# owensgroup/sparsify.me

Measured on AMD Instinct MI355X. Metric: effective GF/s (2:4 spmma vs dense gemm) on ResNet-50 layer shapes, higher is better.
Workload: dtype f16

## Files before the change

sparsify.me_amd/csrc/spmma_f16_fused.hip:

```cpp
#include "select24.h"
#include "spmma_args.h"

namespace sm {

constexpr int MAXG = 8;
struct FusedArgs {
  const half_t* A[MAXG];
  const half_t* B[MAXG];
  half_t* C[MAXG];
  size_t sA, sB, sC;
  int Mrows, N, K, lda;
  int batch, tiles_m, tiles_n;
  int ngroup;
  float alpha, beta;
  const half_t* const* dAp;
  const half_t* const* dBp;
  half_t* const* dCp;
};

template <int BN, int NS, bool BF = false, int BM = 128, int NWV = 4, bool ANT = true, bool DENSE = false>
__global__ __launch_bounds__(64 * NWV, (BN == 128 && NWV == 4 && BM == 128) ? 4 : 1) void spmma_f16_fused_direct_kernel(const FusedArgs p) {
  static_assert(BM == 128 || BM == 64, "row tile");
  static_assert(NWV == 4 || (NWV == 8 && BM == 128), "waves per workgroup");
  constexpr int NW = NWV, TM = BM / NW, FM = TM / 16, FN = BN / 16;
// ... 979 lines not shown
        strip_select_f16(src[i][0], src[i][1], k0, n0);
        strip_select_f16(src[i][2], src[i][3], k1, n1);
        *reinterpret_cast<u2*>(sb + a_val_off[i]) = u2{k0, k1};
        *reinterpret_cast<unsigned char*>(sb + a_meta_off[i]) = (unsigned char)(n0 | (n1 << 4));
      }
    };
    auto step = [&](int g, u4 (&rr)[4], bool write, bool load) {
      asm volatile("s_waitcnt lgkmcnt(0)\n\ts_barrier" ::: "memory");
      __builtin_amdgcn_sched_barrier(0);
      if (write) write_stage(g + 1, rr);
      if (load) load_a(rr);
      __builtin_amdgcn_sched_barrier(0);
    };
    int g0 = 0;
    if (S > 2 * PF) {
#pragma unroll
      for (int s = 0; s < PF; ++s) load_a(ra[s]);
      write_stage(0, ra[0]);
      load_a(ra[0]);
      for (; g0 + 2 * PF < S; g0 += PF) {
#pragma unroll
        for (int u = 0; u < PF; ++u) step(g0 + u, ra[(u + 1) % PF], true, true);
      }
    } else {
#pragma unroll
      for (int s = 0; s < PF; ++s)
        if (s < S) load_a(ra[s]);
      write_stage(0, ra[0]);
      if (PF < S) load_a(ra[0]);
    }
    for (; g0 < S; g0 += PF) {
#pragma unroll
      for (int u = 0; u < PF; ++u) {
        const int g = g0 + u;
        if (g < S) step(g, ra[(u + 1) % PF], g + 1 < S, g + 1 + PF < S);
      }
    }
  } else {
    const unsigned g4 = lane >> 4, r = lane & 15u;
    const unsigned wm = wave / WN, wn = wave % WN;
    char* const patch = smem + CPATCH + wave * WPATCH;
    f4 acc[FM][FN];
#pragma unroll
    for (int i = 0; i < FM; ++i)
#pragma unroll
      for (int j = 0; j < FN; ++j) acc[i][j] = f4{0.f, 0.f, 0.f, 0.f};
    int cb = 0, kt = 0;
    unsigned cj = 0;
    Tile t = tile_of(0);
    for (int g = 0; g < S; ++g) {
      asm volatile("s_barrier" ::: "memory");
      const char* As = smem + (g & 1) * ASTG;
      smfmac_stage<FM, FN, BF>(As, As + SA, smem + BRING + cb * SB, wm * TM, wn * TN, lane, acc);
      cb = cb + 1 == NSB ? 0 : cb + 1;
      if (++kt == nkt) {
        half_t* C = p.C[t.grp] + (size_t)t.b * p.sC;
        const bool c_vec = (reinterpret_cast<uintptr_t>(C) & 15u) == 0 && (p.N % 8 == 0);
        if (p.beta == 0.0f && c_vec) {
#pragma unroll
          for (int h = 0; h < 2; ++h) {
#pragma unroll
            for (int i = 0; i < FM; ++i)
#pragma unroll
              for (int j = 0; j < FN / 2; ++j) {
                const unsigned lr = i * 16 + 4u * g4, lc = j * 16 + r;
#pragma unroll
                for (int q = 0; q < 4; ++q)
                  *reinterpret_cast<half_t*>(patch + (lr + q) * WPITCH + lc * 2) = to_elt<BF>(p.alpha * acc[i][h * (FN / 2) + j][q]);
              }
            asm volatile("s_waitcnt lgkmcnt(0)" ::: "memory");
            const int gc = t.n0 + (int)(wn * TN) + 64 * h + 8 * (int)(lane & 7u);
#pragma unroll
            for (int s8 = 0; s8 < TM / 8; ++s8) {
              const unsigned lr = 8u * s8 + (lane >> 3);
              const int gr = t.m0 + (int)(wm * TM + lr);
              if (gr < p.Mrows && gc < p.N) {
                const u2 lo = *reinterpret_cast<const u2*>(patch + lr * WPITCH + 16u * (lane & 7u));
                const u2 hi = *reinterpret_cast<const u2*>(patch + lr * WPITCH + 16u * (lane & 7u) + 8u);
                __builtin_nontemporal_store(u4{lo[0], lo[1], hi[0], hi[1]}, reinterpret_cast<u4*>(C + (size_t)gr * p.N + gc));
              }
            }
            asm volatile("s_waitcnt lgkmcnt(0)" ::: "memory");
          }
        } else {
#pragma unroll
          for (int i = 0; i < FM; ++i)
#pragma unroll
            for (int j = 0; j < FN; ++j) {
              const int gc = t.n0 + (int)(wn * TN + j * 16 + r);
              if (gc >= p.N) continue;
#pragma unroll
              for (int q = 0; q < 4; ++q) {
                const int gr = t.m0 + (int)(wm * TM + i * 16 + 4u * g4) + q;
                if (gr >= p.Mrows) continue;
                half_t* dst = C + (size_t)gr * p.N + gc;
                float v = p.alpha * acc[i][j][q];
                if (p.beta != 0.0f) v += p.beta * to_f32<BF>(*dst);
                *dst = to_elt<BF>(v);
              }
            }
        }
#pragma unroll
        for (int i = 0; i < FM; ++i)
#pragma unroll
          for (int j = 0; j < FN; ++j) acc[i][j] = f4{0.f, 0.f, 0.f, 0.f};
        kt = 0;
        if (++cj < my_tiles) t = tile_of(cj);
      }
    }
  }
}

template <int BN, int WM, int WN, int NLB, int PF, int NSB, bool BF = false>
static int launch_fused_widep(const FusedArgs& a0, hipStream_t st) {
  FusedArgs a = a0;
  a.tiles_m = (a.Mrows + 127) / 128;
  a.tiles_n = (a.N + BN - 1) / BN;
  const size_t nt = (size_t)a.tiles_m * a.tiles_n * a.batch * a.ngroup;
  if (nt == 0) return SM_STATUS_SUCCESS;
  if (nt > 0x7fffffffu) {
    set_error("sm_spmma_fused_f16: grid too large");
    return SM_STATUS_NOT_SUPPORTED;
  }
  constexpr size_t lds = 2 * (size_t)128 * 72 + (size_t)NSB * 64 * BN * 2 + (size_t)(WM * WN) * 32 * (64 * 2 + 8);
  static_assert(lds <= 160 * 1024, "LDS budget of the persistent wide kernel");
  static LdsOptIn lds_optin;
  if (const int rc = ensure_dyn_lds(lds_optin, reinterpret_cast<const void*>(&spmma_f16_fused_widep_kernel<BN, WM, WN, NLB, PF, NSB, BF>), lds, "spmma_f16_fused_widep_kernel")) return rc;
  size_t cus = (size_t)device_cu_count();
  cus -= cus % 8;
  if (cus == 0) cus = 8;
  const unsigned grid = (unsigned)(nt <= cus ? nt : cus);
  spmma_f16_fused_widep_kernel<BN, WM, WN, NLB, PF, NSB, BF><<<dim3(grid), dim3(64 * (WM * WN + 4 + NLB)), lds, st>>>(a, (unsigned)nt);
  return check_launch("spmma_f16_fused_widep_kernel");
}

template <int NSB, bool BF = false>
__global__ __launch_bounds__(64 * 16) void spmma_f16_fused_astat_kernel(const FusedArgs p, int nsplit, int tiles_per_split) {
  constexpr int BM = 128, BN = 128, WM = 4, WN = 2, NC = 8, NLA = 4, NLB = 4;
  static_assert(NC + NLA + NLB == 16, "launch bounds");
  constexpr int TM = BM / WM, TN = BN / WN, FM = TM / 16, FN = TN / 16;
  constexpr int SA = BM * 64, SM_ = BM * 8, ASTG = SA + SM_, SB = 64 * BN * 2;
  constexpr int B_N = BN / 8, B_WI = B_N / NLB;
  static_assert((NSB - 2) * B_WI <= 63, "vmcnt range");
  constexpr int WPITCH = TN * 2 + 8, WPATCH = TM * WPITCH;
  extern __shared__ __attribute__((aligned(16))) char smem[];

  const unsigned tid = threadIdx.x, lane = tid & 63u;
  const unsigned wave = __builtin_amdgcn_readfirstlane(tid >> 6);
  const int nkt = p.K / 64;
  const unsigned per_batch = (unsigned)p.tiles_m * (unsigned)nsplit;
  const unsigned lid = xcd_remap(blockIdx.x, gridDim.x);
  const unsigned gb = lid / per_batch, trem = lid - gb * per_batch;
  const unsigned grp = gb / (unsigned)p.batch, b = gb - grp * (unsigned)p.batch;
  const unsigned tile_m = trem / (unsigned)nsplit, split = trem - tile_m * (unsigned)nsplit;
  const int m0 = (int)tile_m * BM;
  const int nt0 = (int)split * tiles_per_split;
  const int nt1 = nt0 + tiles_per_split < p.tiles_n ? nt0 + tiles_per_split : p.tiles_n;
  const int T = (nt1 - nt0) * nkt;
  char* const Bring = smem + nkt * ASTG;
  char* const Cpatch = Bring + NSB * SB;
  half_t* C = p.C[grp] + (size_t)b * p.sC;

  const bool is_b = wave >= (unsigned)(NC + NLA);
  const unsigned lwb = is_b ? wave - (NC + NLA) : 0u;
  const char* Bb = reinterpret_cast<const char*>(p.B[grp] + (size_t)b * p.sB);
  unsigned b_kr[B_WI], b_col[B_WI], b_dst[B_WI];
#pragma unroll
  for (int i = 0; i < B_WI; ++i) {
    const unsigned j = lwb + (unsigned)NLB * i, panel = j >> 3, grp = j & 7u, kr = 8u * grp + (lane >> 3);
    b_kr[i] = kr;
    b_col[i] = 64u * panel + 8u * ((lane & 7u) ^ b_swz(kr));
    b_dst[i] = panel * 8192u + grp * 1024u;
  }
  const size_t row_bytes = (size_t)p.N * 2;
  int i_nt = nt0, i_kt = 0, i_buf = 0;
  auto issue_b = [&]() {
#pragma unroll
    for (int i = 0; i < B_WI; ++i) {
      int gc = i_nt * BN + (int)b_col[i];
      gc = gc <= p.N - 8 ? gc : p.N - 8;
      const char* src = Bb + (size_t)(i_kt * 64 + (int)b_kr[i]) * row_bytes + (size_t)gc * 2;
      __builtin_amdgcn_global_load_lds((gptr_t*)src, (lptr_t*)(Bring + i_buf * SB + b_dst[i]), 16, 0, 0);
    }
    i_buf = i_buf + 1 == NSB ? 0 : i_buf + 1;
    if (++i_kt == nkt) { i_kt = 0; ++i_nt; }
  };
  if (is_b) {
#pragma unroll
    for (int s = 0; s < NSB - 1; ++s)
      if (s < T) issue_b();
  }

  {
    const half_t* A = p.A[grp] + (size_t)b * p.sA;
    const unsigned row = 8u * wave + (lane >> 3), c8 = lane & 7u;
    int gr = m0 + (int)row;
    gr = gr < p.Mrows - 1 ? gr : p.Mrows - 1;
    const half_t* a_src = A + (size_t)gr * p.lda + 8u * c8;
    const unsigned a_val_off = row * 64u + 16u * ((c8 >> 1) ^ a64_swz(row)) + 8u * (c8 & 1u);
    const unsigned a_meta_off = SA + row * 8u + c8;
    u4 ra[8];
#pragma unroll
    for (int s = 0; s < 8; ++s)
      if (s < nkt) ra[s] = __builtin_nontemporal_load(reinterpret_cast<const u4*>(a_src + (size_t)s * 64));
#pragma unroll
    for (int s = 0; s < 8; ++s)
      if (s < nkt) {
        uint32_t k0, k1, n0, n1;
        strip_select_f16(ra[s][0], ra[s][1], k0, n0);
        strip_select_f16(ra[s][2], ra[s][3], k1, n1);
        char* sb = smem + s * ASTG;
        *reinterpret_cast<u2*>(sb + a_val_off) = u2{k0, k1};
        *reinterpret_cast<unsigned char*>(sb + a_meta_off) = (unsigned char)(n0 | (n1 << 4));
      }
  }
  __syncthreads();
  if (wave >= (unsigned)NC && !is_b) {
    for (int it = 0; it < T; ++it) asm volatile("s_barrier" ::: "memory");
    return;
  }

  if (is_b) {
    for (int it = 0; it < T; ++it) {
      if (it + NSB - 2 < T) wait_dma_and_barrier<(NSB - 2) * B_WI>();
      else wait_dma_and_barrier<0>();
      if (it + NSB - 1 < T) issue_b();
    }
  } else {
    const unsigned g = lane >> 4, r = lane & 15u;
    const unsigned wm = wave / WN, wn = wave % WN;
    char* const patch = Cpatch + wave * WPATCH;
    f4 acc[FM][FN];
#pragma unroll
    for (int i = 0; i < FM; ++i)
#pragma unroll
      for (int j = 0; j < FN; ++j) acc[i][j] = f4{0.f, 0.f, 0.f, 0.f};
    int cb = 0, kt = 0, nt = nt0;
    for (int it = 0; it < T; ++it) {
      asm volatile("s_barrier" ::: "memory");
      const char* As = smem + kt * ASTG;
      const char* Ms = As + SA;
      const char* Bs = Bring + cb * SB;
      smfmac_stage<FM, FN, BF>(As, Ms, Bs, wm * TM, wn * TN, lane, acc);
      cb = cb + 1 == NSB ? 0 : cb + 1;
      if (++kt == nkt) {
#pragma unroll
        for (int i = 0; i < FM; ++i)
#pragma unroll
          for (int j = 0; j < FN; ++j) {
            const unsigned lr = i * 16 + 4u * g, lc = j * 16 + r;
#pragma unroll
            for (int q = 0; q < 4; ++q) {
              *reinterpret_cast<half_t*>(patch + (lr + q) * WPITCH + lc * 2) = to_elt<BF>(p.alpha * acc[i][j][q]);
              acc[i][j][q] = 0.f;
            }
          }
        asm volatile("s_waitcnt lgkmcnt(0)" ::: "memory");
        const int gc = nt * BN + (int)(wn * TN) + 8 * (int)(lane & 7u);
#pragma unroll
        for (int s = 0; s < TM / 8; ++s) {
          const unsigned lr = 8u * s + (lane >> 3);
          const int gr = m0 + (int)(wm * TM + lr);
          if (gr < p.Mrows && gc < p.N) {
            const u2 lo = *reinterpret_cast<const u2*>(patch + lr * WPITCH + 16u * (lane & 7u));
            const u2 hi = *reinterpret_cast<const u2*>(patch + lr * WPITCH + 16u * (lane & 7u) + 8u);
            __builtin_nontemporal_store(u4{lo[0], lo[1], hi[0], hi[1]}, reinterpret_cast<u4*>(C + (size_t)gr * p.N + gc));
          }
        }
        kt = 0;
        ++nt;
      }
    }
  }
}


static size_t astat_lds_bytes(int nkt, int nsb) { return (size_t)nkt * (128 * 72) + (size_t)nsb * 64 * 128 * 2 + 8 * 32 * (64 * 2 + 8); }

template <bool BF = false>
static int launch_fused_astat(const FusedArgs& a0, hipStream_t st) {
  FusedArgs a = a0;
  a.tiles_m = (a.Mrows + 127) / 128;
  a.tiles_n = (a.N + 127) / 128;
  const int cus = device_cu_count();
  const size_t panels = (size_t)a.tiles_m * a.batch * a.ngroup;
  int nsplit = 1;
  while (panels * nsplit * 4 < (size_t)3 * cus && (a.tiles_n + 2 * nsplit - 1) / (2 * nsplit) >= 2) nsplit *= 2;
  int tps = (a.tiles_n + nsplit - 1) / nsplit;
  nsplit = (a.tiles_n + tps - 1) / tps;
  const size_t nwg = panels * nsplit;
  if (nwg == 0) return SM_STATUS_SUCCESS;
  if (nwg > 0x7fffffffu) {
    set_error("sm_spmma_fused_f16: grid too large");
    return SM_STATUS_NOT_SUPPORTED;
  }
  constexpr int NSB = 3;
  const size_t lds = astat_lds_bytes(a.K / 64, NSB);
  static LdsOptIn lds_optin;
  if (const int rc = ensure_dyn_lds(lds_optin, reinterpret_cast<const void*>(&spmma_f16_fused_astat_kernel<NSB, BF>), (160 * 1024), "spmma_f16_fused_astat_kernel")) return rc;
  spmma_f16_fused_astat_kernel<NSB, BF><<<dim3((unsigned)nwg), dim3(64 * 16), lds, st>>>(a, nsplit, tps);
  return check_launch("spmma_f16_fused_astat_kernel");
}

}

using namespace sm;

static bool span_form_takes(size_t m, size_t n, size_t k, size_t lda, size_t batch, size_t strideA, size_t strideB, size_t strideC, bool all_aligned, bool c_aligned) {
  return (k % 64 != 0 || lda % 8 != 0) && lda == k && n % 8 == 0 && n <= 128 && all_aligned && c_aligned && (batch == 1 || (strideB == 0 && strideA == m * lda && strideC == m * n)) &&
         (m * batch * k * 2) % 16 == 0 && m * batch <= 0x7fffffffull && k <= 0x7fffffffull &&
         ((size_t)128 * k * 2 + 1152) + ((k + 63) / 64 * 64) * (n <= 64 ? 64 : 128) * 2 <= 160 * 1024;
}
static bool stage_forms_take(size_t n, size_t k, size_t lda, size_t strideA, size_t strideB, bool all_aligned) {
  return !(k % 64 != 0 || lda % 8 != 0 || strideA % 8 != 0 || n % 8 != 0 || strideB % 8 != 0 || !all_aligned);
}
static bool dims_fit_int(size_t m, size_t n, size_t k, size_t lda, size_t batch) {
  return !(m * batch > 0x7fffffffull || n > 0x7fffffffull || k > 0x7fffffffull || lda > 0x7fffffffull);
}
bool sm::spmma_fused16_takes_exact(const void* A, const void* B, const void* C, size_t m, size_t n, size_t k, size_t lda, size_t batch, size_t strideA, size_t strideB,
                                   size_t strideC) {
  if (!A || !B || !C || lda < k || m == 0 || n == 0 || batch == 0) return false;
  if (n < 8 && k <= 64) return false;
  const bool all_aligned = aligned16(A) && aligned16(B), c_aligned = aligned16(C);
  if (span_form_takes(m, n, k, lda, batch, strideA, strideB, strideC, all_aligned, c_aligned)) return true;
  return stage_forms_take(n, k, lda, strideA, strideB, all_aligned) && dims_fit_int(m, n, k, lda, batch);
}

template <bool BF>
static int spmma_fused16(size_t ngroup, const void* const* Ag, const void* const* Bg, void* const* Cg, size_t m, size_t n, size_t k, size_t lda,
                         size_t batch, size_t strideA, size_t strideB, size_t strideC, float alpha, float beta,
                         sm_stream_t stream, void* workspace = nullptr, size_t workspace_bytes = 0) {
  if (ngroup == 0) return SM_STATUS_SUCCESS;
  if (!Ag || !Bg || !Cg || lda < k || ngroup > (size_t)MAXG) {
    set_error("sm_spmma_fused_{f16,bf16}: invalid argument");
    return SM_STATUS_INVALID_VALUE;
  }
  bool all_aligned = true, c_aligned = true;
  for (size_t g = 0; g < ngroup; ++g) {
    if (!Ag[g] || !Bg[g] || !Cg[g]) {
      set_error("sm_spmma_fused_{f16,bf16}: invalid argument (null operand)");
      return SM_STATUS_INVALID_VALUE;
    }
    all_aligned = all_aligned && aligned16(Ag[g]) && aligned16(Bg[g]);
    c_aligned = c_aligned && aligned16(Cg[g]);
  }
  if (m == 0 || n == 0 || batch == 0) return SM_STATUS_SUCCESS;
  if (n < 8 && k <= 64 && lda == k && (batch == 1 || (strideB == 0 && strideA == m * lda && strideC == m * n))) {
    const int rc = spmma_fused_thin(BF, (int)ngroup, Ag, Bg, Cg, m * batch, n, k, alpha, beta, (hipStream_t)stream);
    if (rc != SM_STATUS_NOT_SUPPORTED) return rc;
  }
  if (span_form_takes(m, n, k, lda, batch, strideA, strideB, strideC, all_aligned, c_aligned)) {
    FusedArgs a = {};
    for (size_t g = 0; g < (size_t)MAXG; ++g) {
      const size_t s_ = g < ngroup ? g : 0;
      a.A[g] = (const half_t*)Ag[s_]; a.B[g] = (const half_t*)Bg[s_]; a.C[g] = (half_t*)Cg[s_];
    }
    a.ngroup = (int)ngroup;
    a.Mrows = (int)(m * batch); a.N = (int)n; a.K = (int)k; a.lda = (int)lda;
    a.batch = 1; a.alpha = alpha; a.beta = beta;
    hipStream_t st = (hipStream_t)stream;
    return n <= 64 ? launch_fused_span<64, BF>(a, st) : launch_fused_span<128, BF>(a, st);
  }
  if (!stage_forms_take(n, k, lda, strideA, strideB, all_aligned)) {
    set_error("sm_spmma_fused_{f16,bf16}: needs k %% 64 == 0, n %% 8 == 0 and 16-byte aligned rows (use the staged path)");
    return SM_STATUS_NOT_SUPPORTED;
  }
  if (ngroup > 1 && !c_aligned) {
    set_error("sm_spmma_fused_{f16,bf16}_grouped: needs 16-byte aligned C operands");
    return SM_STATUS_NOT_SUPPORTED;
  }
  if (!dims_fit_int(m, n, k, lda, batch)) {
    set_error("sm_spmma_fused_{f16,bf16}: dimension exceeds 2^31-1");
    return SM_STATUS_NOT_SUPPORTED;
  }
  FusedArgs a = {};
  for (size_t g = 0; g < (size_t)MAXG; ++g) {
    const size_t s_ = g < ngroup ? g : 0;
    a.A[g] = (const half_t*)Ag[s_]; a.B[g] = (const half_t*)Bg[s_]; a.C[g] = (half_t*)Cg[s_];
  }
  a.ngroup = (int)ngroup;
  void* const C = Cg[0];
  a.sA = strideA; a.sB = strideB; a.sC = strideC;
  a.Mrows = (int)m; a.N = (int)n; a.K = (int)k; a.lda = (int)lda;
  a.batch = (int)batch; a.alpha = alpha; a.beta = beta;
  if (batch > 1 && strideB == 0 && strideA == m * lda && strideC == m * n) {
    a.Mrows = (int)(m * batch);
    a.batch = 1;
  }
  hipStream_t st = (hipStream_t)stream;
  auto round_eff = [](size_t tiles, size_t cus) { const size_t r = (tiles + cus - 1) / cus; return r ? (double)tiles / (double)(r * cus) : 1.0; };
  if (workspace) {
    const bool astat_shape = n > 256 && k <= 512 && beta == 0.0f && aligned16(C) && (strideC % 8 == 0);
    SkPlan pl;
    if (sk_takes((size_t)a.Mrows, (size_t)a.batch * a.ngroup, n, k, astat_shape, pl) &&
        workspace_bytes >= sk_workspace_bytes((size_t)pl.slots * ((n + 255) / 256), 256) && aligned16(workspace)) {
      const int rc = n <= 256 ? launch_fused_sk<256, BF, true>(a, workspace, workspace_bytes, st) : launch_fused_sk<256, BF, false>(a, workspace, workspace_bytes, st);
      if (rc != SM_STATUS_NOT_SUPPORTED) return rc;
    }
  }
  if (n > 128 && k > 64) {
    const size_t cus = (size_t)device_cu_count(), nb = (size_t)a.batch * a.ngroup;
    const size_t t_big = ((size_t)a.Mrows + 255) / 256 * ((n + 255) / 256) * nb, t_wide = ((size_t)a.Mrows + 127) / 128 * ((n + 255) / 256) * nb;
    const bool astat_shape = n > 256 && k <= 512 && beta == 0.0f && aligned16(C) && (strideC % 8 == 0);
    bool big = round_eff(t_big, cus) >= round_eff(t_wide, cus);
    if (astat_shape) {
      const size_t panels = ((size_t)a.Mrows + 127) / 128 * nb;
      size_t ns = 1, tn = (n + 127) / 128;
      while (panels * ns * 4 < 3 * cus && (tn + 2 * ns - 1) / (2 * ns) >= 2) ns *= 2;
      big = round_eff(t_big, cus) > round_eff(panels * ns, cus) + 0.1;
    }
    if (big) return n <= 256 ? launch_fused_big<256, BF, 3, 2, true>(a, st) : launch_fused_big<256, BF, 3, 2, false>(a, st);
  }
  if (n <= 128 || (n <= 256 && k <= 64)) {
    if (n <= 64) return launch_fused_direct<64, 2, BF>(a, st);
    if (n > 128 || k < 512) return launch_fused_direct<128, 2, BF, 128, 4, false>(a, st);
    return launch_fused_direct<128, 2, BF>(a, st);
  }
  if (n > 256 && k <= 512 && beta == 0.0f && aligned16(C) && (strideC % 8 == 0) &&
      astat_lds_bytes((int)(k / 64), 3) <= 160 * 1024) {
    return launch_fused_astat<BF>(a, st);
  }
  if (k <= 1024) return launch_fused_widep<256, 4, 2, 4, 2, 3, BF>(a, st);
  if (n > 256) return launch_fused_wide<256, 4, 2, 4, 2, 3, BF, false>(a, st);
  return launch_fused_wide<256, 4, 2, 4, 2, 3, BF>(a, st);
}

extern "C" int sm_spmma_fused_f16(const void* A, const void* B, void* C, size_t m, size_t n, size_t k, size_t lda,
                                  size_t batch, size_t strideA, size_t strideB, size_t strideC, float alpha, float beta,
                                  sm_stream_t stream) {
  return spmma_fused16<false>(1, &A, &B, &C, m, n, k, lda, batch, strideA, strideB, strideC, alpha, beta, stream);
}
extern "C" int sm_spmma_fused_bf16(const void* A, const void* B, void* C, size_t m, size_t n, size_t k, size_t lda,
                                   size_t batch, size_t strideA, size_t strideB, size_t strideC, float alpha, float beta,
                                   sm_stream_t stream) {
  return spmma_fused16<true>(1, &A, &B, &C, m, n, k, lda, batch, strideA, strideB, strideC, alpha, beta, stream);
}

extern "C" int sm_spmma_fused_workspace_size(size_t* bytes) {
  if (!bytes) {
    set_error("sm_spmma_fused_workspace_size: invalid argument");
    return SM_STATUS_INVALID_VALUE;
  }
  *bytes = sk_workspace_bytes((size_t)device_cu_count(), 256);
  return SM_STATUS_SUCCESS;
}
extern "C" int sm_spmma_fused_workspace_state(const void* workspace, int* state, sm_stream_t stream) {
  if (!workspace || !state) {
    set_error("sm_spmma_fused_workspace_state: invalid argument");
    return SM_STATUS_INVALID_VALUE;
  }
  unsigned h[1024];
  hipStream_t st = (hipStream_t)stream;
  if (hipMemcpyAsync(h, workspace, sizeof(h), hipMemcpyDeviceToHost, st) != hipSuccess || hipStreamSynchronize(st) != hipSuccess)
    return check_launch("sm_spmma_fused_workspace_state");
  bool dirty = false;
  for (int i = 0; i < 1023; ++i) dirty = dirty || h[i] != 0u;
  *state = h[1023] != 0u ? 1 : (dirty ? 2 : 0);
  return SM_STATUS_SUCCESS;
}
extern "C" int sm_spmma_fused_streamk_plan(size_t rows, size_t n, size_t k, size_t problems, int* takes, unsigned* plan) {
  if (!takes || !plan) {
    set_error("sm_spmma_fused_streamk_plan: invalid argument");
    return SM_STATUS_INVALID_VALUE;
  }
  SkPlan pl = {};
  *takes = sk_takes(rows, problems, n, k, n > 256 && k <= 512, pl) ? 1 : 0;
  unsigned* o = plan;
  *o++ = pl.tg; *o++ = pl.wg; *o++ = pl.groups_full; *o++ = pl.tgl; *o++ = pl.wgl; *o++ = pl.slots; *o++ = pl.units;
  for (int i = 0; i < 9; ++i) *o++ = pl.cut[i];
  for (int i = 0; i < 9; ++i) *o++ = pl.cutl[i];
  return SM_STATUS_SUCCESS;
}
extern "C" int sm_spmma_fused_f16_ws(const void* A, const void* B, void* C, size_t m, size_t n, size_t k, size_t lda, size_t batch, size_t strideA,
                                     size_t strideB, size_t strideC, float alpha, float beta, void* workspace, size_t workspace_bytes, sm_stream_t stream) {
  return spmma_fused16<false>(1, &A, &B, &C, m, n, k, lda, batch, strideA, strideB, strideC, alpha, beta, stream, workspace, workspace_bytes);
}
extern "C" int sm_spmma_fused_bf16_ws(const void* A, const void* B, void* C, size_t m, size_t n, size_t k, size_t lda, size_t batch, size_t strideA,
                                      size_t strideB, size_t strideC, float alpha, float beta, void* workspace, size_t workspace_bytes, sm_stream_t stream) {
  return spmma_fused16<true>(1, &A, &B, &C, m, n, k, lda, batch, strideA, strideB, strideC, alpha, beta, stream, workspace, workspace_bytes);
}

template <bool BF>
static int dense_twin16(const DenseTwinCall& c, hipStream_t st) {
  const size_t n = (size_t)c.N, k = (size_t)c.K;
  const bool tables = c.Ap != nullptr;
  if (tables != (c.Bp != nullptr) || tables != (c.Cp != nullptr)) return SM_STATUS_NOT_SUPPORTED;
  if (c.N % 8 != 0 || c.N < 8 || (!tables && (!aligned16(c.A) || !aligned16(c.B) || !aligned16(c.C)))) return SM_STATUS_NOT_SUPPORTED;
  FusedArgs a = {};
  for (int g = 0; g < MAXG; ++g) { a.A[g] = c.A; a.B[g] = c.B; a.C[g] = c.C; }
  a.dAp = c.Ap; a.dBp = c.Bp; a.dCp = c.Cp;
  a.ngroup = 1;
  a.sA = c.sA; a.sB = c.sB; a.sC = c.sC;
  a.Mrows = c.M; a.N = c.N; a.K = c.K; a.lda = c.lda;
  a.batch = c.batch; a.alpha = c.alpha; a.beta = c.beta;
  if (k % 64 != 0 || c.lda % 8 != 0) {
    if (c.lda != c.K || n > 128 || ((size_t)c.M * k * 2) % 16 != 0 || (c.batch > 1 && !tables)) return SM_STATUS_NOT_SUPPORTED;
    if (((size_t)128 * k * 2 + 1152) + ((k + 63) / 64 * 64) * (n <= 64 ? 64 : 128) * 2 > 160 * 1024) return SM_STATUS_NOT_SUPPORTED;
    a.ngroup = c.batch;
    a.batch = 1;
    if (!tables) a.ngroup = 1;
    return n <= 64 ? launch_fused_span<64, BF, true>(a, st) : launch_fused_span<128, BF, true>(a, st);
  }
  if (c.sA % 8 != 0 || c.sB % 8 != 0) return SM_STATUS_NOT_SUPPORTED;
  if (c.workspace && n > 128 && n <= 256 && k >= 2048) {
    SkPlan pl;
    if (sk_takes((size_t)c.M, (size_t)c.batch, n, k, false, pl) && c.workspace_bytes >= sk_workspace_bytes((size_t)pl.slots * ((n + 255) / 256), 256) &&
        aligned16(c.workspace))
      return launch_fused_sk<256, BF, true, true>(a, c.workspace, c.workspace_bytes, st);
  }
  if (n <= 128) return SM_STATUS_NOT_SUPPORTED;
  if (k <= 64) return SM_STATUS_NOT_SUPPORTED;
  if (((size_t)c.M + 255) / 256 * 256 * 100 > (size_t)c.M * 115) return SM_STATUS_NOT_SUPPORTED;
  if (!(n <= 256 && k >= 2048)) return SM_STATUS_NOT_SUPPORTED;
  return launch_fused_big<256, BF, 3, 2, true, true>(a, st);
}

int sm::gemm_dense_twin(const DenseTwinCall& c, hipStream_t st) { return c.bf ? dense_twin16<true>(c, st) : dense_twin16<false>(c, st); }

template <bool BF>
static int spmma_fused16_grouped(size_t count, const void* const* A, const void* const* B, void* const* C, size_t m, size_t n, size_t k,
                                 size_t lda, size_t batch, size_t strideA, size_t strideB, size_t strideC, float alpha, float beta,
                                 sm_stream_t stream, void* workspace = nullptr, size_t workspace_bytes = 0) {
  if (count && (!A || !B || !C)) {
    set_error("sm_spmma_fused_{f16,bf16}_grouped: invalid argument");
    return SM_STATUS_INVALID_VALUE;
  }
  for (size_t i = 0; i < count; i += (size_t)MAXG) {
    const size_t ng = count - i < (size_t)MAXG ? count - i : (size_t)MAXG;
    if (const int rc = spmma_fused16<BF>(ng, A + i, B + i, C + i, m, n, k, lda, batch, strideA, strideB, strideC, alpha, beta, stream, workspace, workspace_bytes)) return rc;
  }
  return SM_STATUS_SUCCESS;
}
extern "C" int sm_spmma_fused_f16_grouped(size_t count, const void* const* A, const void* const* B, void* const* C, size_t m, size_t n,
                                          size_t k, size_t lda, size_t batch, size_t strideA, size_t strideB, size_t strideC,
                                          float alpha, float beta, sm_stream_t stream) {
  return spmma_fused16_grouped<false>(count, A, B, C, m, n, k, lda, batch, strideA, strideB, strideC, alpha, beta, stream);
}
extern "C" int sm_spmma_fused_bf16_grouped(size_t count, const void* const* A, const void* const* B, void* const* C, size_t m, size_t n,
                                           size_t k, size_t lda, size_t batch, size_t strideA, size_t strideB, size_t strideC,
                                           float alpha, float beta, sm_stream_t stream) {
  return spmma_fused16_grouped<true>(count, A, B, C, m, n, k, lda, batch, strideA, strideB, strideC, alpha, beta, stream);
}
extern "C" int sm_spmma_fused_f16_grouped_ws(size_t count, const void* const* A, const void* const* B, void* const* C, size_t m, size_t n,
                                             size_t k, size_t lda, size_t batch, size_t strideA, size_t strideB, size_t strideC,
                                             float alpha, float beta, void* workspace, size_t workspace_bytes, sm_stream_t stream) {
  return spmma_fused16_grouped<false>(count, A, B, C, m, n, k, lda, batch, strideA, strideB, strideC, alpha, beta, stream, workspace, workspace_bytes);
}
extern "C" int sm_spmma_fused_bf16_grouped_ws(size_t count, const void* const* A, const void* const* B, void* const* C, size_t m, size_t n,
                                              size_t k, size_t lda, size_t batch, size_t strideA, size_t strideB, size_t strideC,
                                              float alpha, float beta, void* workspace, size_t workspace_bytes, sm_stream_t stream) {
  return spmma_fused16_grouped<true>(count, A, B, C, m, n, k, lda, batch, strideA, strideB, strideC, alpha, beta, stream, workspace, workspace_bytes);
}
```

Measured before the change: 572,100.

## Add A-stationary expand kernel with DMA producer wave for wide-N short-K shapes

Adds a new fused 2:4 sparse kernel for n>256, k<=512 and beta==0. Each workgroup compresses a 256-row A panel once into registers, and a dedicated fifth wave streams 64-column B chunks into LDS through global_load_lds with multi-stage buffering. Four compute waves run smfmac sweeps and write C directly, using DPP and ds_swizzle shuffles to assemble 16-byte row stores. The path replaces the previous big/astat selection for these shapes. The cost is high register pressure from holding all K fragments, a new N-split heuristic, and a template instance per K/64.

```diff
diff --git a/sparsify.me_amd/csrc/spmma_f16_fused.hip b/sparsify.me_amd/csrc/spmma_f16_fused.hip
--- a/sparsify.me_amd/csrc/spmma_f16_fused.hip
+++ b/sparsify.me_amd/csrc/spmma_f16_fused.hip
@@ -1305,6 +1305,185 @@
   return check_launch("spmma_f16_fused_astat_kernel");
 }
 
+template <int NKT>
+struct ExpandCfg {
+  static constexpr int NS = NKT <= 2 ? 3 : 2;
+  static constexpr int CHUNK = NKT * 8192;
+  static constexpr int LDS = NS * CHUNK;
+  static constexpr int WAVES_PER_EU = NKT <= 4 ? 3 : 2;
+};
+
+__device__ __forceinline__ uint32_t swz_xor4(uint32_t v) { return (uint32_t)__builtin_amdgcn_ds_swizzle((int)v, 0x101F); }
+__device__ __forceinline__ uint32_t dpp_xor2(uint32_t v) { return (uint32_t)__builtin_amdgcn_mov_dpp((int)v, 0x4E, 0xF, 0xF, true); }
+__device__ __forceinline__ uint32_t dpp_xor1(uint32_t v) { return (uint32_t)__builtin_amdgcn_mov_dpp((int)v, 0xB1, 0xF, 0xF, true); }
+
+template <bool BF>
+__device__ __forceinline__ u2 frag_rows(const f4 v, float alpha, unsigned u) {
+  const uint32_t v01 = (uint32_t)__builtin_bit_cast(unsigned short, to_elt<BF>(alpha * v[0])) |
+                       ((uint32_t)__builtin_bit_cast(unsigned short, to_elt<BF>(alpha * v[1])) << 16);
+  const uint32_t v23 = (uint32_t)__builtin_bit_cast(unsigned short, to_elt<BF>(alpha * v[2])) |
+                       ((uint32_t)__builtin_bit_cast(unsigned short, to_elt<BF>(alpha * v[3])) << 16);
+  const uint32_t r2 = dpp_xor2((u & 2u) ? v01 : v23);
+  const uint32_t P = (u & 2u) ? r2 : v01, Q = (u & 2u) ? v23 : r2;
+  const bool odd = (u & 1u) != 0u;
+  const uint32_t r1 = dpp_xor1(odd ? ((P & 0xffffu) | (Q << 16)) : ((P >> 16) | (Q & 0xffff0000u)));
+  return odd ? u2{(r1 & 0xffffu) | (P & 0xffff0000u), (r1 >> 16) | (Q & 0xffff0000u)}
+             : u2{(P & 0xffffu) | (r1 << 16), (Q & 0xffffu) | (r1 & 0xffff0000u)};
+}
+
+template <int NKT, bool BF = false>
+__global__ __launch_bounds__(64 * 5, ExpandCfg<NKT>::WAVES_PER_EU) void spmma_f16_fused_expand_kernel(const FusedArgs p, int nsplit, int chunks_per_split) {
+  using Cfg = ExpandCfg<NKT>;
+  constexpr int NS = Cfg::NS, CHUNK = Cfg::CHUNK, FM = 4, BM = 256;
+  constexpr int PIECES = NKT * 8;
+  static_assert(NS == 2 || (NS - 2) * PIECES <= 63, "vmcnt range");
+  extern __shared__ __attribute__((aligned(16))) char smem[];
+
+  const unsigned tid = threadIdx.x, lane = tid & 63u;
+  const unsigned wave = __builtin_amdgcn_readfirstlane(tid >> 6);
+  const unsigned per_batch = (unsigned)p.tiles_m * (unsigned)nsplit;
+  const unsigned lid = xcd_remap(blockIdx.x, gridDim.x);
+  const unsigned gb = lid / per_batch, trem = lid - gb * per_batch;
+  const unsigned grp = gb / (unsigned)p.batch, b = gb - grp * (unsigned)p.batch;
+  const unsigned tile_m = trem / (unsigned)nsplit, split = trem - tile_m * (unsigned)nsplit;
+  const int m0 = (int)tile_m * BM;
+  const int ch0 = (int)split * chunks_per_split;
+  const int ch1 = ch0 + chunks_per_split < p.tiles_n ? ch0 + chunks_per_split : p.tiles_n;
+  const int T = ch1 - ch0;
+
+  if (wave == 4) {
+    const char* Bb = reinterpret_cast<const char*>(p.B[grp] + (size_t)b * p.sB);
+    const size_t row_bytes = (size_t)p.N * 2;
+    auto issue = [&](int c) {
+      char* dst = smem + (c % NS) * CHUNK;
+#pragma unroll
+      for (int j = 0; j < 8; ++j) {
+        const unsigned kr = 8u * j + (lane >> 3);
+        int gc = (ch0 + c) * 64 + 8 * (int)((lane & 7u) ^ b_swz(kr));
+        gc = gc <= p.N - 8 ? gc : p.N - 8;
+        const char* src = Bb + (size_t)kr * row_bytes + (size_t)gc * 2;
+#pragma unroll
+        for (int s = 0; s < NKT; ++s)
+          __builtin_amdgcn_global_load_lds((gptr_t*)(src + (size_t)s * 64 * row_bytes), (lptr_t*)(dst + s * 8192 + j * 1024), 16, 0, 0);
+      }
+    };
+#pragma unroll
+    for (int c = 0; c < NS - 1; ++c)
+      if (c < T) issue(c);
+    for (int c = 0; c < T; ++c) {
+      if (NS > 2 && c + NS - 2 < T) wait_dma_and_barrier<(NS > 2 ? (NS - 2) * PIECES : 0)>();
+      else wait_dma_and_barrier<0>();
+      if (c + NS - 1 < T) issue(c + NS - 1);
+    }
+    return;
+  }
+
+  const unsigned g = lane >> 4, r = lane & 15u, t = (lane >> 2) & 3u, u = lane & 3u;
+  h8 af[NKT][FM];
+  int idx[NKT][FM];
+  {
+    const half_t* A = p.A[grp] + (size_t)b * p.sA;
+    const half_t* arow[FM];
+#pragma unroll
+    for (int i = 0; i < FM; ++i) {
+      int gr = m0 + (int)(wave * 64u + 16u * i + r);
+      gr = gr < p.Mrows - 1 ? gr : p.Mrows - 1;
+      arow[i] = A + (size_t)gr * p.lda + 16u * g;
+    }
+    constexpr int EA = 3;
+    u4 raw[EA][FM][2];
+    auto load = [&](int s) {
+      int ks = s * 64;
+      asm volatile("" : "+v"(ks));
+#pragma unroll
+      for (int i = 0; i < FM; ++i) {
+        raw[s % EA][i][0] = *reinterpret_cast<const u4*>(arow[i] + ks);
+        raw[s % EA][i][1] = *reinterpret_cast<const u4*>(arow[i] + ks + 8);
+      }
+    };
+#pragma unroll
+    for (int s = 0; s < EA; ++s)
+      if (s < NKT) load(s);
+#pragma unroll
+    for (int s = 0; s < NKT; ++s) {
+#pragma unroll
+      for (int i = 0; i < FM; ++i) dense16_to_operand(raw[s % EA][i][0], raw[s % EA][i][1], af[s][i], idx[s][i]);
+      if (s + EA < NKT) load(s + EA);
+    }
+  }
+  half_t* C = p.C[grp] + (size_t)b * p.sC;
+  const int row_l = (int)(wave * 64u + 4u * g + u);
+  const int col_l = (int)(4u * (t & 2u) + 16u * (t & 1u));
+  for (int c = 0; c < T; ++c) {
+    asm volatile("s_barrier" ::: "memory");
+    const char* Bs = smem + (c % NS) * CHUNK;
+#pragma unroll
+    for (int h = 0; h < 2; ++h) {
+      f4 acc[FM][2];
+#pragma unroll
+      for (int i = 0; i < FM; ++i) acc[i][0] = acc[i][1] = f4{0.f, 0.f, 0.f, 0.f};
+#pragma unroll
+      for (int s = 0; s < NKT; ++s) smfmac_b_sweep<FM, 2, BF>(af[s], idx[s], Bs + s * 8192, 32u * h, lane, acc);
+      const int gc = (ch0 + c) * 64 + 32 * h + col_l;
+#pragma unroll
+      for (int i = 0; i < FM; ++i) {
+        const u2 x0 = frag_rows<BF>(acc[i][0], p.alpha, u), x1 = frag_rows<BF>(acc[i][1], p.alpha, u);
+        const bool odd = (t & 1u) != 0u;
+        const uint32_t s0 = swz_xor4(odd ? x0[0] : x1[0]), s1 = swz_xor4(odd ? x0[1] : x1[1]);
+        const u4 v = odd ? u4{s0, s1, x1[0], x1[1]} : u4{x0[0], x0[1], s0, s1};
+        const int gr = m0 + row_l + 16 * i;
+        if (gr < p.Mrows && gc < p.N) *reinterpret_cast<u4*>(C + (size_t)gr * p.N + gc) = v;
+      }
+    }
+  }
+}
+
+template <int NKT, bool BF>
+static int launch_fused_expand_nkt(const FusedArgs& a, int nsplit, int cps, size_t nwg, hipStream_t st) {
+  constexpr size_t lds = ExpandCfg<NKT>::LDS;
+  static LdsOptIn lds_optin;
+  if (lds > 64 * 1024) {
+    if (const int rc = ensure_dyn_lds(lds_optin, reinterpret_cast<const void*>(&spmma_f16_fused_expand_kernel<NKT, BF>), lds, "spmma_f16_fused_expand_kernel")) return rc;
+  }
+  spmma_f16_fused_expand_kernel<NKT, BF><<<dim3((unsigned)nwg), dim3(64 * 5), lds, st>>>(a, nsplit, cps);
+  return check_launch("spmma_f16_fused_expand_kernel");
+}
+
+static size_t expand_lds_bytes(int nkt) { return (size_t)(nkt <= 2 ? 3 : 2) * nkt * 8192; }
+
+template <bool BF = false>
+static int launch_fused_expand(const FusedArgs& a0, hipStream_t st) {
+  FusedArgs a = a0;
+  a.tiles_m = (a.Mrows + 255) / 256;
+  a.tiles_n = (a.N + 63) / 64;
+  const size_t per_cu = expand_lds_bytes(a.K / 64) <= 80 * 1024 ? 2 : 1;
+  const size_t slots = (size_t)device_cu_count() * per_cu;
+  const size_t panels = (size_t)a.tiles_m * a.batch * a.ngroup;
+  auto round_eff = [&](size_t wg) { const size_t r = (wg + slots - 1) / slots; return r ? (double)wg / (double)(r * slots) : 1.0; };
+  int nsplit = 1;
+  while (round_eff(panels * nsplit) < 0.85 && a.tiles_n >= 4 * nsplit) nsplit *= 2;
+  const int cps = (a.tiles_n + nsplit - 1) / nsplit;
+  nsplit = (a.tiles_n + cps - 1) / cps;
+  const size_t nwg = panels * nsplit;
+  if (nwg == 0) return SM_STATUS_SUCCESS;
+  if (nwg > 0x7fffffffu) {
+    set_error("sm_spmma_fused_f16: grid too large");
+    return SM_STATUS_NOT_SUPPORTED;
+  }
+  switch (a.K / 64) {
+    case 1: return launch_fused_expand_nkt<1, BF>(a, nsplit, cps, nwg, st);
+    case 2: return launch_fused_expand_nkt<2, BF>(a, nsplit, cps, nwg, st);
+    case 3: return launch_fused_expand_nkt<3, BF>(a, nsplit, cps, nwg, st);
+    case 4: return launch_fused_expand_nkt<4, BF>(a, nsplit, cps, nwg, st);
+    case 5: return launch_fused_expand_nkt<5, BF>(a, nsplit, cps, nwg, st);
+    case 6: return launch_fused_expand_nkt<6, BF>(a, nsplit, cps, nwg, st);
+    case 7: return launch_fused_expand_nkt<7, BF>(a, nsplit, cps, nwg, st);
+    case 8: return launch_fused_expand_nkt<8, BF>(a, nsplit, cps, nwg, st);
+  }
+  set_error("sm_spmma_fused_f16: expand form needs 64 <= k <= 512");
+  return SM_STATUS_NOT_SUPPORTED;
+}
+
 }
 
 using namespace sm;
@@ -1401,6 +1580,7 @@
       if (rc != SM_STATUS_NOT_SUPPORTED) return rc;
     }
   }
+  if (n > 256 && k <= 512 && beta == 0.0f && aligned16(C) && (strideC % 8 == 0)) return launch_fused_expand<BF>(a, st);
   if (n > 128 && k > 64) {
     const size_t cus = (size_t)device_cu_count(), nb = (size_t)a.batch * a.ngroup;
     const size_t t_big = ((size_t)a.Mrows + 255) / 256 * ((n + 255) / 256) * nb, t_wide = ((size_t)a.Mrows + 127) / 128 * ((n + 255) / 256) * nb;
```

Result: slower. 366,800 (median of 2 runs) (-35.9%).
